# ChalmersPhotonicsLab/QAMpy

Hardware: AMD Instinct MI355X
Metric: equalised MSym/s (2-pol, 2 SPS) (higher is better)
Workload: dtype f32

## Files before the change

### qampy_amd/csrc/api.hip

```cpp
#include "common.h"
#include <stdlib.h>
#include <atomic>
#include <mutex>
#include <vector>
#include <unordered_map>
#include <string.h>

namespace qh {

thread_local hipStream_t g_stream = nullptr;
static thread_local hipStream_t g_streams[4] = {nullptr, nullptr, nullptr, nullptr};
int g_device = -1;
static thread_local std::string g_err;
static std::mutex g_mu;

void set_error(const std::string &s) { g_err = s; }

int hip_fail(hipError_t e, const char *what, const char *file, int line)
{
    g_err = std::string(hipGetErrorString(e)) + " in " + what + " (" + file + ":" + std::to_string(line) + ")";
    (void)hipGetLastError();
    return QH_ERR_HIP;
}

// ... 63 lines not shown
        QH_HIP(hipStreamCreateWithPriority(&g_streams[i], hipStreamNonBlocking, i == 2 ? prio_least : prio_greatest));
    }
    g_stream = g_streams[0];
    g_device = device;
    return QH_OK;
}

hipStream_t side_stream() { return g_stream == g_streams[0] ? g_streams[1] : g_streams[0]; }
hipStream_t helper_stream() { return g_streams[3]; }

int ensure_init()
{
    if (g_stream) return QH_OK;
    return init_device(g_device >= 0 ? g_device : 0);
}

thread_local void *g_scratch[SCRATCH_SLOTS] = {nullptr};
thread_local size_t g_scratch_n[SCRATCH_SLOTS] = {0};
thread_local unsigned g_scratch_epoch = 0;
static std::atomic<int> g_form[FORM_COUNT];
struct FormName { const char *key, *env; };
static const FormName FORM_NAMES[FORM_COUNT] = {
    {"trainer", "QAMPY_HIP_TRAINER"}, {"pit_form", "QAMPY_HIP_PIT_FORM"}, {"seg_lanes", "QAMPY_HIP_SEG_LANES"}, {"pit_probe", "QAMPY_HIP_PIT_PROBE"},
    {"bps", "QAMPY_HIP_BPS"}};
static int form_parse(int k, const char *v, int *out)
{
    if (!v || !v[0]) { *out = 0; return 0; }
    switch (k) {
    case FORM_TRAINER: *out = v[0] == 'd' ? 1 : (v[0] == 'l' ? 2 : (v[0] == 'i' ? 3 : (v[0] == 'a' || v[0] == '0' ? 0 : -1))); break;
    case FORM_PIT: *out = v[0] == 's' ? 1 : (v[0] == 'b' ? 2 : (v[0] == 'a' || v[0] == '0' ? 0 : -1)); break;
    case FORM_SEG_LANES: { const int n = atoi(v); *out = (n == 8 || n == 16 || n == 0) ? n : -1; break; }
    case FORM_BPS: *out = v[0] == 't' ? 1 : (v[0] == 'l' ? 2 : (v[0] == 'a' || v[0] == '0' ? 0 : -1)); break;
    default: *out = atoi(v) != 0 ? 1 : 0; break;
    }
    return *out < 0 ? -1 : 0;
}
static const int g_form_env_read = [] {
    for (int k = 0; k < FORM_COUNT; k++) {
        int v = 0;
        if (form_parse(k, getenv(FORM_NAMES[k].env), &v) == 0) g_form[k].store(v);
    }
    return 0;
}();
int form(FormKey k) { return g_form[k].load(std::memory_order_relaxed); }
const char *trainer_force()
{
    switch (form(FORM_TRAINER)) {
    case 1: return "direct";
    case 2: return "lookahead";
    case 3: return "iterative";
    default: return "";
    }
}
static constexpr int POOL_CLASSES = 48, POOL_KEEP = 8;
static constexpr size_t POOL_BYTES = (size_t)24 << 30;
// ... 370 lines not shown
```

### qampy_amd/csrc/common.h

```cpp
#pragma once
#include <hip/hip_runtime.h>
#include <stdint.h>
#include <string>
#include "../../include/qampy_hip.h"

namespace qh {

extern thread_local hipStream_t g_stream;
extern int g_device;
void set_error(const std::string &s);
int hip_fail(hipError_t e, const char *what, const char *file, int line);

#define QH_HIP(call)                                                        \
    do {                                                                    \
        hipError_t _e = (call);                                             \
        if (_e != hipSuccess) return qh::hip_fail(_e, #call, __FILE__, __LINE__); \
    } while (0)

#define QH_REQUIRE(cond, msg)                                   \
    do {                                                        \
        if (!(cond)) { qh::set_error(msg); return QH_ERR_ARG; } \
    } while (0)

#define QH_WAVE_FIRST() __builtin_amdgcn_s_setprio(3)

int ensure_init();
hipStream_t side_stream();
hipStream_t helper_stream();
enum FormKey { FORM_TRAINER = 0, FORM_PIT, FORM_SEG_LANES, FORM_PIT_PROBE, FORM_BPS, FORM_COUNT };
int form(FormKey k);
const char *trainer_force();
double gram_budget_gb();
int pit_timing_mode();
int default_tier();
double default_tier_tol();
constexpr int SCRATCH_SLOTS = 24;
constexpr int SCRATCH_TWOSTAGE = 16;
constexpr int SCRATCH_FOE = 17;
constexpr int SCRATCH_IMPAIR = 18;
constexpr int SCRATCH_PMD = 19;
constexpr int SCRATCH_TXRESP = 20;
constexpr int SCRATCH_SOS = 21;
constexpr int SCRATCH_CPR = 22;
constexpr int SCRATCH_FFT = 23;
int scratch(int slot, size_t bytes, void **p);
unsigned scratch_epoch();

int bps_twostage_recover_f32(const void *E, int nm, int64_t L, const void *angles, int A, int B, const void *symbols, int M, int N, int32_t *idx1,
                             int32_t *idx2, void *ph, void *Eout);
int bps_twostage_recover_f64(const void *E, int nm, int64_t L, const void *angles, int A, int B, const void *symbols, int M, int N, int32_t *idx1,
                             int32_t *idx2, void *ph, void *Eout);

// ... 114 lines not shown
```

### qampy_amd/csrc/train_pit.h

```cpp
#pragma once
#include <atomic>
#include <chrono>
#include <vector>
#include "train_impl.h"
#include "train_seg.h"

namespace qh {

typedef qh_pit_report PitCtrl;

constexpr double PIT_CONTRACT = 0.2;
constexpr int PIT_PROBE = 128;
constexpr int PIT_SEEDWIN = 512;
constexpr int PIT_MAXSEG = 65536;

__host__ __device__ inline int pit_symmetry(int method)
{
    switch (method) {
    case QH_M_CMA: case QH_M_SGNCMA: case QH_M_RDE: return 0;
    case QH_M_CMA2: return 2;
    default: return 4;
    }
}

// ... 832 lines not shown
                if (q < n) {
                    const float4 g = gch[rr * npair + lane];
                    const Zf up = row[p];
                    const Zf xqe = cmulf(Zf{g.z, -g.w}, row[q]);
                    row[p] = Zf{g.x * up.x - g.y * xqe.x, g.x * up.y - g.y * xqe.y};
                    row[q] = Zf{g.y * up.x + g.x * xqe.x, g.y * up.y + g.x * xqe.y};
                }
            }
            __builtin_amdgcn_fence(__ATOMIC_RELEASE, "wavefront");
        }
    }
    for (int k = lane; k < n; k += 64) { Vout[(size_t)i * n + k] = row[k]; Vout[(size_t)n * n + (size_t)k * n + i] = row[k]; }
}

constexpr int PIT_GT = 16, PIT_GC = PIT_GT / 8;
template <typename R> struct PitFuse {
    Cx<R> *X, *Y;
    const double *theta;
    const int64_t *modes_dev;
    int nmodes, nsel;
    float damp = 1.f;
    const Cx<R> *T2 = nullptr;
    float2 *Out2 = nullptr;
};
template <typename R, bool CONJT>
__global__ void __launch_bounds__(256) pit_cgemm_kernel(const Zf *A2, const Zf *B, Zf *C, int n, int ncol, const PitCtrl *c, PitFuse<R> fz)
{
    QH_WAVE_FIRST();
    if (c->done) return;
    extern __shared__ __attribute__((aligned(16))) char pit_smem[];
    Zf *As = reinterpret_cast<Zf *>(pit_smem);
    Zf *Bs = As + (size_t)PIT_EIGMAX * PIT_EIGMAX;
    const int tx = threadIdx.x & 7, ty = threadIdx.x >> 3;
    const int col0 = blockIdx.x * PIT_GT;
    const size_t wset = (size_t)fz.nmodes * n;
    for (int e = threadIdx.x; e < PIT_EIGMAX * n; e += 256) {
        const int k = e / PIT_EIGMAX, m = e - k * PIT_EIGMAX;
        Zf v{0.f, 0.f};
        if (m < n) { v = A2[(size_t)k * n + m]; if (CONJT) v.y = -v.y; }
        As[e] = v;
    }
    if (CONJT) {
        for (int e = threadIdx.x; e < n * PIT_GT; e += 256) {
            const int cc = e / n, k = e - cc * n, col = col0 + cc;
            Zf v{0.f, 0.f};
            if (col < ncol) {
// ... 233 lines not shown
            }
        } else if (threadIdx.x == 0) {
            float k11 = vals[0], k12 = vals[1], k22 = vals[2], zz = vals[3];
            const float cs = vals[4];
            const float n = cs > 0.f ? 1.f / cs : 0.f;
            k11 *= n; k12 *= n; k22 *= n; zz *= n;
            const float tr = 0.5f * (k11 + k22), df = 0.5f * (k11 - k22), rad = sqrtf(df * df + k12 * k12);
            float c = 1.f, sn = 0.f;
            if (rad > 1e-12f * (fabsf(tr) + 1e-30f)) { const float ang = 0.5f * atan2f(k12, df); c = cosf(ang); sn = sinf(ang); }
            PitModel m = a.model[j];
            m.k1 = tr + rad; m.k2 = tr - rad; m.q11 = c; m.q21 = sn; m.q12 = -sn; m.q22 = c; m.lam_u = zz;
            m.ok = (m.g > 0.f && m.g == m.g && m.k1 == m.k1 && m.k2 == m.k2) ? 1 : 0;
            a.model[j] = m;
        }
        __syncthreads();
    }
}

typedef float pit_f4 __attribute__((ext_vector_type(4)));
constexpr int PIT_MC = 16, PIT_MBP = PIT_MC + 1;
inline int pit_mfma_threads(int n) { return 64 * ((n + 15) / 16); }
inline size_t pit_mfma_lds(int n) { return ((size_t)(n + 4) * PIT_MBP + (size_t)PIT_MC * (PIT_EIGMAX + 1)) * sizeof(Zf); }
template <typename R, int MODE>
__global__ void __launch_bounds__(64 * (PIT_EIGMAX / 16)) pit_basis_mfma_kernel(const Zf *__restrict__ A2, const Cx<R> *__restrict__ T, const Zf *__restrict__ D, Zf *__restrict__ Out,
                                                                               int n, int ncol, const PitCtrl *c, PitFuse<R> fz)
{
    QH_WAVE_FIRST();
    if (c->done) return;
    extern __shared__ __attribute__((aligned(16))) char pit_smem[];
    const int np = (n + 3) & ~3;
    Zf *Bs = reinterpret_cast<Zf *>(pit_smem);
    Zf *Ct = Bs + (size_t)(n + 4) * PIT_MBP;
    const int tid = threadIdx.x, lane = tid & 63, wave = tid >> 6, nw = blockDim.x >> 6, nt = blockDim.x;
    const int nb1 = (ncol + PIT_MC - 1) / PIT_MC;
    const bool second = MODE == 0 && (int)blockIdx.x >= nb1;
    if (second) { T = fz.T2; Out = reinterpret_cast<Zf *>(fz.Out2); }
    const int col0 = ((int)blockIdx.x - (second ? nb1 : 0)) * PIT_MC;
    const size_t wset = (size_t)fz.nmodes * n;
    const int am = 16 * wave + (lane & 15), ak = lane >> 4;
    const Zf *ag = A2 + (size_t)ak * n + am;
    auto lda = [&](int k) -> Zf { return (am < n && k + ak < n) ? ag[(size_t)k * n] : Zf{0.f, 0.f}; };
    constexpr int PF = 8;
    Zf abuf[PF];
#pragma unroll
    for (int i = 0; i < PF; i++) abuf[i] = lda(4 * i);
    constexpr int NCW = 3;
    if (MODE == 0) {
        for (int cb = 0; cb < PIT_MC; cb += NCW * nw) {
            Zf tmp[NCW][2];
#pragma unroll
            for (int q = 0; q < NCW; q++) {
                const int cc = cb + wave + nw * q, col = col0 + cc;
                tmp[q][0] = Zf{0.f, 0.f}; tmp[q][1] = Zf{0.f, 0.f};
                if (cc < PIT_MC && col < ncol) {
                    const int s = col / fz.nsel, j = col - s * fz.nsel;
                    const Cx<R> *src = T + (size_t)s * wset + (size_t)fz.modes_dev[j] * n;
                    if (lane < n) { const Cx<R> t = src[lane]; tmp[q][0] = Zf{(float)t.re, (float)t.im}; }
                    if (lane + 64 < n) { const Cx<R> t = src[lane + 64]; tmp[q][1] = Zf{(float)t.re, (float)t.im}; }
                }
            }
// ... 70 lines not shown
    } else {
#pragma unroll
        for (int q = 0; q < 4; q++) {
            const int m = 16 * wave + 4 * (lane >> 4) + q;
            Ct[cl * (PIT_EIGMAX + 1) + m] = Zf{rr[q] - ii[q], im[q]};
        }
        __syncthreads();
        for (int cb = 0; cb < PIT_MC; cb += NCW * nw) {
#pragma unroll
            for (int q = 0; q < NCW; q++) {
                const int cc = cb + wave + nw * q, col = col0 + cc;
                if (cc < PIT_MC && col < ncol) {
                    const int s = col / fz.nsel, j = col - s * fz.nsel;
                    const size_t base = (size_t)s * wset + (size_t)fz.modes_dev[j] * n;
                    const double qr = pre ? th[q][0] : fz.theta[2 * (size_t)col], qi = pre ? th[q][1] : fz.theta[2 * (size_t)col + 1];
#pragma unroll
                    for (int h = 0; h < 2; h++) {
                        const int m = lane + 64 * h;
                        if (m < n) {
                            const Cx<R> x = pre ? xv[q][h] : fz.X[base + m];
                            const Zf d = Ct[cc * (PIT_EIGMAX + 1) + m];
                            const Cx<R> w{(R)(qr * x.re - qi * x.im + fz.damp * d.x), (R)(qr * x.im + qi * x.re + fz.damp * d.y)};
                            fz.X[base + m] = w;
                            fz.Y[base + m] = w;
                        }
                    }
                }
            }
        }
    }
}

static __global__ void __launch_bounds__(256) pit_bound_kernel(const Zf *Xe, const Zf *Ye, const Zf *Yprev, const double *lam, int n, int S, int nsel, int sym,
                                                              const PitCtrl *c, double *dfc, double *pw, double *gph, float4 *ualpha = nullptr)
{
    QH_WAVE_FIRST();
    if (c->done) return;
    const int lane = threadIdx.x & 63, bi = blockIdx.x * 4 + (threadIdx.x >> 6);
    const int nb = (S - 1) * nsel, ncol = S * nsel;
    if (bi >= nb + nsel) return;
    const bool result_probe = bi >= nb;
    const int j = result_probe ? bi - nb : bi % nsel;
    const int sb = result_probe ? S - 1 : bi / nsel;
    const Zf *pa = result_probe ? (c->passes == 0 ? Xe + (size_t)(S - 1) * nsel + j : Yprev + j) : Xe + (size_t)(sb + 1) * nsel + j;
    const size_t sa = (result_probe && c->passes != 0) ? (size_t)nsel : (size_t)ncol;
    const Zf *pb = Ye + (size_t)sb * nsel + j;
    Zf av[(PIT_EIGMAX + 63) / 64], bv[(PIT_EIGMAX + 63) / 64];
    float lv[(PIT_EIGMAX + 63) / 64];
    double A = 0, B = 0, Cr = 0, Ci = 0;
#pragma unroll
    for (int q = 0; q < (PIT_EIGMAX + 63) / 64; q++) {
        const int k = lane + 64 * q;
        av[q] = Zf{0.f, 0.f}; bv[q] = Zf{0.f, 0.f}; lv[q] = 0.f;
// ... 396 lines not shown
                const int s = s0 + q;
                run = cm(run, g[j][q]);
                if (s < s1) {
                    const double r = rsqrt(run.x * run.x + run.y * run.y);
                    th2[(size_t)s * nsel + j] = double2{run.x * r, run.y * r};
                }
            }
        }
        return;
    }
    for (int j = 0; j < nsel; j++) {
        double2 prod{1.0, 0.0};
        for (int s = s0; s < s1; s++)
            if (s > 0) prod = cm(prod, g2[(size_t)(s - 1) * nsel + j]);
        double2 run = block_scan_excl<double2, decltype(cm), NT>(prod, cm, double2{1.0, 0.0}, gbuf);
        for (int s = s0; s < s1; s++) {
            if (s > 0) run = cm(run, g2[(size_t)(s - 1) * nsel + j]);
            const double r = rsqrt(run.x * run.x + run.y * run.y);
            th2[(size_t)s * nsel + j] = double2{run.x * r, run.y * r};
        }
    }
}
template <typename R>
__global__ void __launch_bounds__(256) pit_devest_kernel(const Zf *D, const double *lam, int n, int ncol, const PitCtrl *c, float *devmax, unsigned *ticket, PitDecideArgs<R> da)
{
    QH_WAVE_FIRST();
    if (c->done) return;
    __shared__ float part[2][4][64], red[64], reds[64], redt[64], redm[64];
    const int cl = threadIdx.x & 63, kg = threadIdx.x >> 6;
    const int col = blockIdx.x * 64 + cl;
    float acc = 0.f, tap = 0.f;
    if (col < ncol) {
#pragma unroll 8
        for (int k = kg; k < n; k += 4) {
            const Zf v = D[(size_t)k * ncol + col];
            const float l = (float)lam[k], m2 = v.x * v.x + v.y * v.y;
            acc += (l > 0.f ? l : 0.f) * m2;
            tap += m2;
        }
    }
    part[0][kg][cl] = acc; part[1][kg][cl] = tap;
    __syncthreads();
    if (kg == 0) {
        acc = (part[0][0][cl] + part[0][1][cl]) + (part[0][2][cl] + part[0][3][cl]);
        tap = (part[1][0][cl] + part[1][1][cl]) + (part[1][2][cl] + part[1][3][cl]);
        red[cl] = (acc == acc) ? acc : 3.0e38f;
        reds[cl] = (acc == acc) ? acc : 3.0e38f;
        redt[cl] = (tap == tap) ? tap : 3.0e38f;
        redm[cl] = (tap == tap) ? tap : 3.0e38f;
    }
    __syncthreads();
    for (int s = 32; s > 0; s >>= 1) {
        if (threadIdx.x < s) {
            red[threadIdx.x] = red[threadIdx.x] > red[threadIdx.x + s] ? red[threadIdx.x] : red[threadIdx.x + s];
            reds[threadIdx.x] += reds[threadIdx.x + s];
            redt[threadIdx.x] += redt[threadIdx.x + s];
            redm[threadIdx.x] = redm[threadIdx.x] > redm[threadIdx.x + s] ? redm[threadIdx.x] : redm[threadIdx.x + s];
        }
        __syncthreads();
    }
    if (threadIdx.x == 0) {
        devmax[4 * blockIdx.x] = red[0]; devmax[4 * blockIdx.x + 1] = reds[0]; devmax[4 * blockIdx.x + 2] = redt[0]; devmax[4 * blockIdx.x + 3] = redm[0];
    }
    __shared__ int last;
    if (threadIdx.x == 0) {
        __threadfence();
        const unsigned t = atomicAdd(ticket, 1u);
        last = t == gridDim.x - 1;
        if (last) { *ticket = 0; __threadfence(); }
    }
    __syncthreads();
    if (!last) return;
    pit_decide_body<R>(da);
}
static __global__ void __launch_bounds__(256) pit_front_kernel(const Zf *D, const double *lam, int n, int ncol, double thr, int *front, int *bad)
{
    QH_WAVE_FIRST();
    const int col = blockIdx.x * 256 + threadIdx.x;
    if (col >= ncol) return;
    float acc = 0.f;
    for (int k = 0; k < n; k++) { const Zf v = D[(size_t)k * ncol + col]; const float l = (float)lam[k]; acc += (l > 0.f ? l : 0.f) * (v.x * v.x + v.y * v.y); }
    if (!(acc == acc) || acc > 1e30f) { atomicMax(bad, 1); return; }
    if ((double)acc > thr) atomicMax(front, col);
}
struct PitTiming { int npass; float pass_ms[QH_PIT_MAXPASS]; float acq_ms; };
inline PitTiming &pit_timing() { static thread_local PitTiming t; return t; }
constexpr int PIT_NEV = (QH_PIT_MAXPASS > QH_PIT_MAXCHUNK ? QH_PIT_MAXPASS : QH_PIT_MAXCHUNK) + 1;
struct PitEvents { hipEvent_t t0[PIT_NEV], t1[PIT_NEV], flag[PIT_NEV]; int32_t *hflag; float *hview; bool ok; };
inline PitEvents &pit_events()
{
    static thread_local PitEvents e = {{nullptr}, {nullptr}, {nullptr}, nullptr, nullptr, false};
    if (!e.ok) {
        for (int i = 0; i < PIT_NEV; i++) { (void)hipEventCreate(&e.t0[i]); (void)hipEventCreate(&e.t1[i]); (void)hipEventCreateWithFlags(&e.flag[i], hipEventDisableTiming); }
        (void)hipHostMalloc((void **)&e.hflag, PIT_NEV * sizeof(int32_t), hipHostMallocDefault);
        (void)hipHostMalloc((void **)&e.hview, 2 * PIT_NEV * sizeof(float), hipHostMallocCoherent);
        e.ok = e.hflag != nullptr && e.hview != nullptr;
// ... 395 lines not shown
    if (prepared) QH_REQUIRE(seg_form && o.acq_chunk > 0, "train_equaliser: a prepared acquisition belongs to throughput-form passes with acq_chunk given (qh_pit_prepare_*_dev said so)");
    if (block_form && !G && (!seg_form || amax > 0) && !prepared) {
        const int64_t n = seg_form ? pl.ngram : TrSyms;
        rc = pair_tab ? gram_build<R>(E, nmodes, L, os, ntaps, n, &G) : gram_cur_build<R>(E, nmodes, L, os, ntaps, n, &G);
        if (rc) return rc;
    }
    const int64_t g_per_step = pair_tab ? LA_B : GRAM_TRI / 2 / LA_B;

    const int ncol = sg.S * nsel;
    const double *lam = nullptr;
    const Zf *Vb = nullptr;
    Zf *Dz[2] = {nullptr, nullptr};
    Zf *Xe = nullptr, *Ye = nullptr, *Yprev = nullptr;
    if (want_corr) {
        void *cb = nullptr;
        if ((rc = scratch(10, pit_basis_bytes(ntot) + 4 * (size_t)ntot * ncol * sizeof(Zf) + (size_t)ntot * nsel * sizeof(Zf) + 256, &cb))) return rc;
        void *basis = o.basis ? o.basis : cb;
        if (!o.basis && (rc = pit_basis<R>(E, nmodes, L, os, ntaps, TrSyms, basis))) return rc;
        lam = (const double *)basis; Vb = (const Zf *)((const char *)basis + (size_t)ntot * sizeof(double));
        Dz[0] = (Zf *)((char *)cb + (pit_basis_bytes(ntot) + 63) / 64 * 64); Dz[1] = Dz[0] + (size_t)ntot * ncol;
        Xe = Dz[1] + (size_t)ntot * ncol; Ye = Xe + (size_t)ntot * ncol; Yprev = Ye + (size_t)ntot * ncol;
    }
    const bool eig = want_corr && sizeof(R) == 4 && form(FORM_PIT_PROBE) == 0;
    const bool tables_ok = method == QH_M_CMA || method == QH_M_SGNCMA || method == QH_M_MCMA || method == QH_M_RDE || method == QH_M_MRDE ||
                           (decision && (use_bi || seg_form));
    const bool ssb = eig && tables_ok && method != QH_M_CMA2;
    PitModel *model = nullptr;
    float4 *ualpha = nullptr;
    float2 *uqv = nullptr;
    PitModelArgs<R> ma;
    hipEvent_t model_event = nullptr;
    if (ssb) {
        void *mb = nullptr;
        const size_t pw_ = 2 * PIT_EIGMAX + 8;
        const size_t b_part = (size_t)PIT_MODB * 4 * nsel * pw_ * sizeof(float), b_u = ((size_t)nsel * ntot * sizeof(Cx<R>) + 63) / 64 * 64;
        const size_t b_ua = ((size_t)ncol * sizeof(float4) + 63) / 64 * 64, b_uq = ((size_t)ncol * sizeof(float2) + 63) / 64 * 64;
        if ((rc = scratch(14, b_part + b_u + b_ua + b_uq + 16 * sizeof(PitModel) + 128, &mb))) return rc;
        ma.part = (float *)mb; ma.u = (Cx<R> *)((char *)mb + b_part);
        ualpha = (float4 *)((char *)mb + b_part + b_u); uqv = (float2 *)((char *)ualpha + b_ua);
        model = (PitModel *)((char *)uqv + b_uq); ma.model = model; ma.ticket = (unsigned *)(model + 16);
        init.z[1] = ma.ticket; init.zn[1] = sizeof(unsigned);
        init.z[2] = ualpha; init.zn[2] = (unsigned)(b_ua + b_uq);
        ma.E = (const Cx<R> *)E; ma.wx = (const Cx<R> *)wx; ma.L = L; ma.TrSyms = TrSyms; ma.nmodes = nmodes; ma.ntaps = ntaps; ma.os = os; ma.nsel = nsel; ma.method = method;
        if (decision) { ma.symbols = (const Cx<R> *)f.dd_table; ma.nsy = 2 * f.dd_npart + 1; ma.sy_pitch = 2 * BI_DD_MAXLEV; ma.tables = 1; }
        else { ma.symbols = (const Cx<R> *)symbols; ma.nsy = nsy; ma.sy_pitch = nsy; ma.tables = (method == QH_M_RDE || method == QH_M_MRDE) ? 1 : 0; }
        for (int j = 0; j < 16; j++) ma.modes[j] = j < nsel ? modes[j] : 0;
        if (o.corr_beta < 0) beta = 0.0;
    }
    const size_t glds = ((size_t)PIT_EIGMAX * PIT_EIGMAX + (size_t)PIT_EIGMAX * PIT_GT) * sizeof(Zf);
    static std::atomic<bool> gemm_attr{false};
    if (want_corr && !gemm_attr.load(std::memory_order_acquire)) {
        QH_HIP(hipFuncSetAttribute((const void *)pit_cgemm_kernel<R, true>, hipFuncAttributeMaxDynamicSharedMemorySize, 160 * 1024 - 256));
        QH_HIP(hipFuncSetAttribute((const void *)pit_cgemm_kernel<R, false>, hipFuncAttributeMaxDynamicSharedMemorySize, 160 * 1024 - 256));
        QH_HIP(hipFuncSetAttribute((const void *)pit_basis_mfma_kernel<R, 0>, hipFuncAttributeMaxDynamicSharedMemorySize, 128 * 1024));
        QH_HIP(hipFuncSetAttribute((const void *)pit_basis_mfma_kernel<R, 1>, hipFuncAttributeMaxDynamicSharedMemorySize, 128 * 1024));
        gemm_attr.store(true, std::memory_order_release);
    }

    LaArgs<R> la = la_args<R>(E, L, nmodes, ntaps, os, modes, nsel, method, symbols, nsy, mu_dev, err, TrSyms * Niter);
    la.G = (const GramPair<R> *)G; la.gpair = pair_tab ? 1 : 0; la.wx_cs = (int64_t)wset;
    la.dd_general = f.dd_general;
    f.alphabet(la);
    const TrainArgs<R> ta = train_args<R>(E, L, nmodes, ntaps, os, TrSyms, Niter, modes, nsel, method, symbols, nsy, mu_dev, err);

    PitTiming &tm = pit_timing();
    tm.npass = 0; tm.acq_ms = 0;
    bool acq_timed = false;
    PitEvents &ev = pit_events();
    QH_REQUIRE(ev.ok, "train_equaliser: no pinned memory for the pass flags");
    const bool redo_ok = o.exact_redo_off == 0;
    bool fell_back = false;
    if (redo_ok && !adaptive) { init.cd[0] = w_call; init.cs[0] = wx; init.cn[0] = (unsigned)wbytes; }
    if (o.acquire && Niter > 0) { init.cd[1] = w_start; init.cs[1] = wx; init.cn[1] = (unsigned)wbytes; }
    hipLaunchKernelGGL(pit_init_kernel, dim3(32), dim3(256), 0, g_stream, init);
    QH_HIP(hipGetLastError());
    for (int it = 0; it < Niter; it++) {
        if (it == 0 && prepared) {
            const PitPrepLayout lay = pit_prep_layout<R>(nmodes, ntaps, amax);
// ... 42 lines not shown
            static thread_local hipEvent_t ev_seed = nullptr, ev_model = nullptr;
            if (!ev_seed) { QH_HIP(hipEventCreateWithFlags(&ev_seed, hipEventDisableTiming)); QH_HIP(hipEventCreateWithFlags(&ev_model, hipEventDisableTiming)); }
            hipStream_t ss = helper_stream();
            QH_HIP(hipEventRecord(ev_seed, g_stream));
            QH_HIP(hipStreamWaitEvent(ss, ev_seed, 0));
            hipLaunchKernelGGL((pit_model_kernel<R, 0>), dim3(PIT_MODB), dim3(256), 0, ss, ma);
            hipLaunchKernelGGL((pit_model_kernel<R, 1>), dim3(PIT_MODB), dim3(256), 0, ss, ma);
            QH_HIP(hipEventRecord(ev_model, ss));
            model_event = ev_model;
        }
        QH_HIP(hipGetLastError());
        const int timing_mode = pit_timing_mode();
        auto decide_args = [&](int p, const float *dm, const float2 *ye, float2 *yprev, int ne, int ncol_e, int corr_wanted) {
            PitDecideArgs<R> d;
            d.dfc = dfc; d.pw = pw; d.nb = (int)((sg.S - 1) * nsel); d.Ylast = (const Cx<R> *)(Y + (size_t)(sg.S - 1) * wset); d.n = (int)wset; d.wx = (Cx<R> *)wx; d.c = ctrl;
            d.host_view = &ev.hview[2 * p]; d.nrow = nsel; d.devmax = dm; d.ndev = ndev; d.safety = safety; d.Ye = ye; d.Yprev = yprev; d.ne = ne; d.ncol_e = ncol_e;
            d.theta = theta; d.modes_dev = (const int64_t *)modes_dev; d.ntot_w = ntot; d.S = (int)sg.S; d.sym = sym; d.corr_wanted = corr_wanted;
            d.extra = adaptive ? (const float *)ad_chg : nullptr;
            d.Dfin = (ye && !adaptive) ? (const float2 *)Dz[1] : nullptr; d.Vfin = (const float2 *)Vb; d.lam_fin = lam;
            d.stall_from = o.correction == 0 ? QH_PIT_MAXPASS : (adaptive ? 5 : 2);
            return d;
        };
        auto timed = [&](int p) { return timing_mode == 2 || (timing_mode == 1 && p == 1); };
        auto enqueue_pass = [&](int p) -> int {
            ((volatile float *)ev.hview)[2 * p] = -1.f;
            PitFuse<R> fz;
            fz.X = X; fz.Y = Y; fz.theta = theta; fz.modes_dev = (const int64_t *)modes_dev; fz.nmodes = nmodes; fz.nsel = nsel;
            fz.damp = (adaptive && p > 1) ? ad_damp : 1.f;
            if (p > 0 && want_corr) {
                if (eig)
                    hipLaunchKernelGGL((pit_basis_mfma_kernel<R, 1>), dim3((ncol + PIT_MC - 1) / PIT_MC), dim3(pit_mfma_threads(ntot)), pit_mfma_lds(ntot), g_stream, Vb + (size_t)ntot * ntot,
                                       (const Cx<R> *)nullptr, (const Zf *)Dz[1], (Zf *)nullptr, ntot, ncol, (const PitCtrl *)ctrl, fz);
                else
                    hipLaunchKernelGGL((pit_cgemm_kernel<R, false>), dim3((ncol + PIT_GT - 1) / PIT_GT), dim3(256), glds, g_stream, Vb + (size_t)ntot * ntot, (const Zf *)Dz[1], (Zf *)nullptr, ntot, ncol, (const PitCtrl *)ctrl, fz);
                QH_HIP(hipGetLastError());
            } else if (p > 0) {
                QH_HIP(hipMemcpyAsync(X + wset, Y, (size_t)(sg.S - 1) * wbytes, hipMemcpyDeviceToDevice, g_stream));
                QH_HIP(hipMemcpyAsync(Y, X, (size_t)sg.S * wbytes, hipMemcpyDeviceToDevice, g_stream));
            }
            if (o.on_pass) {
                hipStream_t keep = g_stream;
                o.on_pass(o.on_pass_user, it, p);
                g_stream = keep;
            }
            if (timed(p)) QH_HIP(hipEventRecord(ev.t0[p], g_stream));
            if (seg_form) {
                SegArgs<R> sa{};
                sa.E = (const Cx<R> *)E; sa.wx = Y; sa.symbols = la.symbols; sa.err = (Cx<R> *)err; sa.mu = mu_dev;
                sa.L = L; sa.TrSyms = TrSyms; sa.nsy = la.nsy; sa.sy_pitch = la.sy_pitch; sa.err_pitch = TrSyms * Niter; sa.err_off = (int64_t)it * TrSyms;
                sa.nmodes = nmodes; sa.ntaps = ntaps; sa.os = os; sa.nsel = nsel; sa.S = sg.S;
                sa.seg_len = sg.len; sa.seg_extra = sg.extra; sa.seg_tail = sg.tail; sa.seg_begin = sg.begin;
                sa.r_in = ad_rS; sa.r_out = ad_rE; sa.e_in = ad_eS; sa.e_out = ad_eE; sa.mu_sum = (R *)ad_M; sa.adapt_first = sg.begin > 0 ? 1 : 0;
                for (int j = 0; j < 16; j++) sa.modes[j] = j < nsel ? modes[j] : 0;
                sa.skip = &ctrl->done;
                sa.q_first = own_first * nsel; sa.q_count = split ? own_count * nsel : 0;
                pit_last_launch().form = 1;
                if (!split || own_count > 0) { int r = launch_seg<R>(sa, method, adaptive); if (r) return r; }
                if (adaptive) hipLaunchKernelGGL((pit_adapt_scan_kernel<R>), dim3(1), dim3(1024), 0, g_stream, ad_rS, (const R *)ad_rE, ad_eS, (const Cx<R> *)ad_eE, sg.S, ad_chg, (const PitCtrl *)ctrl, ad_relax, ad_rP, ad_dP, ad_newton);
            } else if (block_form) {
                LaArgs<R> ls = la;
                ls.TrSyms = sg.len; ls.nch = sg.S; ls.wx = Y; ls.err_off = (int64_t)it * TrSyms; ls.seg = 1; ls.seg_extra = sg.extra; ls.seg_tail = sg.tail;
                ls.skip = &ctrl->done;
                pit_last_launch() = PitLaunch{use_bi ? 2 : 3, 0, 0, 0, 0, 0};
                if (sg.begin > 0) {
                    ls.E = (const Cx<R> *)E + sg.begin * os; ls.L = L - sg.begin * os; ls.err_off += sg.begin;
                    ls.G = (const GramPair<R> *)G + sg.begin * g_per_step;
                }
                { int r = use_bi ? launch_bi<R>(ls) : launch_la<R>(ls); if (r) return r; }
            } else {
                TrainArgs<R> ts = ta;
                ts.wx = Y; ts.nseg = sg.S; ts.seg_begin = sg.begin; ts.seg_len = sg.len; ts.seg_extra = sg.extra; ts.seg_tail = sg.tail; ts.seg_iter = it; ts.skip = &ctrl->done;
// ... 9 lines not shown
                if (o.exchange(o.exchange_user, Y, (size_t)sg.S * wbytes) != 0) { set_error("train_equaliser: the exchange callback failed"); return QH_ERR_ARG; }
            }
            const int nbnd = (int)((sg.S - 1) * nsel);
            if (eig) {
                if (o.basis && pit_basis_sync().pending) {
                    QH_HIP(hipStreamWaitEvent(g_stream, pit_basis_sync().out, 0));
                    pit_basis_sync().pending = false;
                }
                auto forward2 = [&](const Cx<R> *src, Zf *dst, const Cx<R> *src2, Zf *dst2) {
                    PitFuse<R> f2 = fz;
                    f2.T2 = src2; f2.Out2 = reinterpret_cast<float2 *>(dst2);
                    hipLaunchKernelGGL((pit_basis_mfma_kernel<R, 0>), dim3(2 * ((ncol + PIT_MC - 1) / PIT_MC)), dim3(pit_mfma_threads(ntot)), pit_mfma_lds(ntot), g_stream, Vb, src, (const Zf *)nullptr, dst, ntot, ncol, (const PitCtrl *)ctrl, f2);
                };
                if (p == 0 && model_event) QH_HIP(hipStreamWaitEvent(g_stream, model_event, 0));
                forward2((const Cx<R> *)X, Xe, (const Cx<R> *)Y, Ye);
                hipLaunchKernelGGL(pit_bound_kernel, dim3((nbnd + nsel + 3) / 4), dim3(256), 0, g_stream, (const Zf *)Xe, (const Zf *)Ye, (const Zf *)Yprev, lam, ntot, sg.S, nsel, sym,
                                   (const PitCtrl *)ctrl, dfc, pw, gph, ualpha);
                hipLaunchKernelGGL((pit_gauge_kernel<R>), dim3(ssb ? 2 : 1), dim3(PIT_GT_THREADS), 0, g_stream, (const double *)gph, sg.S, nsel, ctrl, theta, (const double *)pw,
                                   nbnd, method, (const Cx<R> *)symbols + (size_t)modes[0] * nsy, 1, (const PitModel *)model, (const float4 *)ualpha, uqv,
                                   (const R *)mu_dev, sg.len, (const float *)ad_M);
                hipLaunchKernelGGL((pit_recur_eig_kernel<R>), dim3(ntot, nsel), dim3(PIT_RT), 0, g_stream, Xe, (const Zf *)Ye, Dz[1], (const double *)theta, lam, nsel, sg.S, sg.len,
                                   (const R *)mu_dev, beta, (const PitCtrl *)ctrl, (const float *)ad_M, (adaptive && p >= 1) ? ad_damp : 1.f,
                                   (const float4 *)ualpha, (const float2 *)uqv);
                hipLaunchKernelGGL((pit_devest_kernel<R>), dim3(ndev), dim3(256), 0, g_stream, (const Zf *)Dz[1], lam, ntot, ncol, (const PitCtrl *)ctrl, devmax, ticket,
                                   decide_args(p, (const float *)devmax, (const float2 *)Ye, (float2 *)Yprev, ntot, ncol, 1));
            } else {
            const size_t dlds = (2 * (size_t)ntot + (size_t)nmodes * os * pit_phase_pitch(ntaps, os, PIT_PROBE)) * sizeof(Cx<R>);
            QH_REQUIRE(dlds <= 60 * 1024, "train_equaliser: boundary probe does not fit the LDS for this filter shape");
            hipLaunchKernelGGL((pit_defect_kernel<R>), dim3(sg.S, nsel), dim3(PIT_PROBE), dlds, g_stream, (const Cx<R> *)E, nmodes, L, os,
                               ntaps, sg, TrSyms, (const int64_t *)modes_dev, (const Cx<R> *)X, (const Cx<R> *)Y, sym, (const PitCtrl *)ctrl, dfc, pw, gph, (const Cx<R> *)wx);
            hipLaunchKernelGGL((pit_gauge_kernel<R>), dim3(1), dim3(PIT_GT_THREADS), 0, g_stream, (const double *)gph, sg.S, nsel, ctrl, theta, (const double *)pw,
                               nbnd, method, (const Cx<R> *)symbols + (size_t)modes[0] * nsy, want_corr ? 1 : 0);
            if (want_corr) {
                if (o.basis && pit_basis_sync().pending) {
                    QH_HIP(hipStreamWaitEvent(g_stream, pit_basis_sync().out, 0));
                    pit_basis_sync().pending = false;
                }
                hipLaunchKernelGGL((pit_cgemm_kernel<R, true>), dim3((ncol + PIT_GT - 1) / PIT_GT), dim3(256), glds, g_stream, Vb, (const Zf *)nullptr, Dz[1], ntot, ncol, (const PitCtrl *)ctrl, fz);
                hipLaunchKernelGGL((pit_recur_kernel<R>), dim3(ntot, nsel), dim3(256), 0, g_stream, Dz[1], lam, nsel, sg.S, sg.len, (const R *)mu_dev, beta, (const PitCtrl *)ctrl);
                hipLaunchKernelGGL((pit_devest_kernel<R>), dim3(ndev), dim3(256), 0, g_stream, (const Zf *)Dz[1], lam, ntot, ncol, (const PitCtrl *)ctrl, devmax, ticket,
                                   decide_args(p, (const float *)devmax, (const float2 *)nullptr, (float2 *)nullptr, 0, 0, 1));
            } else
                hipLaunchKernelGGL((pit_decide_kernel<R>), dim3(1), dim3(256), 0, g_stream, decide_args(p, (const float *)nullptr, (const float2 *)nullptr, (float2 *)nullptr, 0, 0, 0));
            }
            QH_HIP(hipGetLastError());
            return QH_OK;
// ... 157 lines not shown
```

### qampy_amd/csrc/train_seg.h

```cpp
#pragma once
#include "train_bi.h"

namespace qh {

constexpr int SG_CH = 64;

template <typename R> struct SegArgs {
    const Cx<R> *E;
    Cx<R> *wx;
    const Cx<R> *symbols;
    Cx<R> *err;
    const R *mu;
    int64_t L, TrSyms, nsy, sy_pitch, err_pitch, err_off;
    int nmodes, ntaps, os, nsel, S;
    int64_t seg_len, seg_extra, seg_tail, seg_begin;
    int64_t modes[16];
    const int *skip;
    int q_first, q_count;
    int lpm, pitch, rag, nslots;
    int ch;
    const R *r_in; R *r_out; const Cx<R> *e_in; Cx<R> *e_out; R *mu_sum; int adapt_first;
};

__device__ __forceinline__ void row16_csum(float &re, float &im)
{
    asm volatile(
        "s_nop 1\n\t"
        "v_add_f32_dpp %0, %0, %0 quad_perm:[1,0,3,2] row_mask:0xf bank_mask:0xf\n\t"
        "v_add_f32_dpp %1, %1, %1 quad_perm:[1,0,3,2] row_mask:0xf bank_mask:0xf\n\t"
        "s_nop 0\n\t"
        "v_add_f32_dpp %0, %0, %0 quad_perm:[2,3,0,1] row_mask:0xf bank_mask:0xf\n\t"
        "v_add_f32_dpp %1, %1, %1 quad_perm:[2,3,0,1] row_mask:0xf bank_mask:0xf\n\t"
// ... 253 lines not shown
    const int nq = a.q_count > 0 ? a.q_first + a.q_count : a.S * a.nsel;
    const int q0 = a.q_first + blockIdx.x * CPW;
    const int q = q0 + lane / LPC;
    const bool alive = q < nq;
    const int qc = alive ? q : nq - 1;
    const int seg = qc / a.nsel, jsel = qc - seg * a.nsel;
    const int seg0 = q0 / a.nsel;
    const int segl = ((q0 + CPW - 1 < nq ? q0 + CPW - 1 : nq - 1)) / a.nsel;
    const int nslot = segl - seg0 + 1;
    const int slot = seg - seg0;
    const int mode = (int)a.modes[jsel];
    const int ntot = a.nmodes * a.ntaps;
    const int os_ = a.os;
    auto seg_start = [&](int64_t s) { return a.seg_begin + s * a.seg_len + (s < a.seg_extra ? s : a.seg_extra) * LA_B; };
    auto seg_steps = [&](int64_t s) { return (int)(a.seg_len + (s < a.seg_extra ? LA_B : 0) + (s == a.S - 1 ? a.seg_tail : 0)); };
    const int64_t my_start = seg_start(seg);
    const int my_steps = alive ? seg_steps(seg) : 0;
    int max_steps = 0, min_steps = 0x7fffffff;
    for (int s = seg0; s <= segl; s++) { const int n = seg_steps(s); max_steps = n > max_steps ? n : max_steps; min_steps = n < min_steps ? n : min_steps; }
    if (q0 + CPW - 1 >= nq) min_steps = 0;

    const int kin = l16 / a.lpm, t0 = (l16 - kin * a.lpm) * TPL;
    const bool has = kin < a.nmodes;
    Cx<R> *wrow = a.wx + ((size_t)seg * a.nmodes + mode) * ntot;
    v2 w[TPL];
#pragma unroll
    for (int j = 0; j < TPL; j++) {
        const bool ok = has && t0 + j < a.ntaps;
        const Cx<R> v = ok ? wrow[kin * a.ntaps + t0 + j] : Cx<R>{0, 0};
        w[j] = v2{v.re, v.im};
    }
    const Cx<R> *sy = a.symbols + (size_t)mode * a.sy_pitch;
    LaConst<R, NPART> K;
    K.mu = *a.mu;
    { const Cx<R> c0 = sy[0]; K.R_re = c0.re; K.R_im = c0.im; }
    K.code0_re = K.R_re; K.code0_im = K.R_im;
    tab_fill<R, NPART>(K.tab, sy, 0, NPART + 1);
    LaConst<R, NPART> Ks = K;
    Ks.code0_re *= K.mu; Ks.code0_im *= K.mu;
    tab_scale_codes<R, NPART>(Ks.tab, K.mu);
    R ad_r = 1, ad_sum = 0;
    Cx<R> ad_ep{0, 0};
    bool ad_skip0 = false;
    if constexpr (ADAPT) { ad_r = a.r_in[qc]; ad_ep = a.e_in[qc]; ad_skip0 = a.adapt_first == 0 && my_start == 0; }

    constexpr int rowsz = PITCH;
    constexpr int bufsz = SG_ROWS * PITCH;
// ... 225 lines not shown
        if (c + 1 < nchunk) stage_load(c + 1);
        const Cx<R> *xs = has ? lds + (slot * a.nmodes + kin) * rowsz + t0 : zero_row;
        const int xstep = has ? os_ : 0;
        const int ibase = c * CH;
        const int nst = (max_steps - ibase) < CH ? (max_steps - ibase) : CH;
        auto run2 = [&](auto RG, auto OS2) __attribute__((always_inline)) {
            if (ibase + nst <= min_steps) run_chunk(xs, xstep, ibase, nst, SgInt<0>{}, RG, OS2);
            else run_chunk(xs, xstep, ibase, nst, SgInt<1>{}, RG, OS2);
        };
        auto run = [&](auto RG) __attribute__((always_inline)) {
            if (os_ == 2) run2(RG, SgInt<1>{}); else run2(RG, SgInt<0>{});
        };
        switch (rag) {
        case 0: run(SgInt<0>{}); break;
        case 1: run(SgInt<1>{}); break;
        case 2: run(SgInt<(TPL > 2 ? 2 : 0)>{}); break;
        default: run(SgInt<(TPL > 3 ? 3 : 0)>{}); break;
        }
        __syncthreads();
        if (c + 1 < nchunk) stage_store(c + 1);
        __syncthreads();
    }
    if (alive) {
#pragma unroll
        for (int j = 0; j < TPL; j++)
            if (has && t0 + j < a.ntaps) stg(wrow + kin * a.ntaps + t0 + j, Cx<R>{w[j].x, w[j].y});
        if constexpr (ADAPT) if (l16 == 0) { a.r_out[q] = ad_r; a.e_out[q] = ad_ep; a.mu_sum[q] = ad_sum; }
    }
}

#endif

inline int seg_tpl(int nmodes, int ntaps, int lpc = 16)
{
    for (int tpl : {2, 4, 6, 8, 11}) {
        if (lpc == 16 ? tpl == 11 : (tpl != 6 && tpl != 11)) continue;
        const int lpm = (ntaps + tpl - 1) / tpl;
        if (nmodes * lpm <= lpc && lpm * tpl - ntaps <= SG_MAXRAG && lpm * tpl - ntaps < tpl) return tpl;
    }
    return 0;
}
inline int seg_slots(int nsel, int cpw = 4)
{
    int n = 1;
    for (int q0 = 0; q0 <= cpw * nsel; q0 += cpw) { const int m = (q0 + cpw - 1) / nsel - q0 / nsel + 1; n = m > n ? m : n; }
    return n;
}
inline bool seg_supported(int method, int nmodes, int ntaps, int os, int64_t nsy, size_t elem, int nsel = 1, int rows = 4)
{
// ... 163 lines not shown
```

Before: 1202.

## Fuse PIT deviation-estimate and next-pass basis product into one tail kernel

Adds a pit_tail_kernel that runs the devest reduction/decide blocks and the next pass's MFMA basis-product blocks in a single launch. When this path is active, the next pass skips its separate basis launch. The basis product writes only X, and the segment kernel reads weights from X and writes its results to Y, which removes a duplicate Y store. This saves one launch and one serialization point per pass. The trade-off is that the basis product is now computed speculatively before the decide step, and the launch uses a larger block size with big LDS for all blocks, which may lower occupancy for the devest blocks.

New measurement: 1240, median of 6. 3.2% higher.

```diff
diff --git a/qampy_amd/csrc/api.hip b/qampy_amd/csrc/api.hip
--- a/qampy_amd/csrc/api.hip
+++ b/qampy_amd/csrc/api.hip
@@ -109,7 +109,7 @@
 struct FormName { const char *key, *env; };
 static const FormName FORM_NAMES[FORM_COUNT] = {
     {"trainer", "QAMPY_HIP_TRAINER"}, {"pit_form", "QAMPY_HIP_PIT_FORM"}, {"seg_lanes", "QAMPY_HIP_SEG_LANES"}, {"pit_probe", "QAMPY_HIP_PIT_PROBE"},
-    {"bps", "QAMPY_HIP_BPS"}};
+    {"bps", "QAMPY_HIP_BPS"}, {"pit_tail", "QAMPY_HIP_PIT_TAIL"}};
 static int form_parse(int k, const char *v, int *out)
 {
     if (!v || !v[0]) { *out = 0; return 0; }
@@ -118,6 +118,7 @@
     case FORM_PIT: *out = v[0] == 's' ? 1 : (v[0] == 'b' ? 2 : (v[0] == 'a' || v[0] == '0' ? 0 : -1)); break;
     case FORM_SEG_LANES: { const int n = atoi(v); *out = (n == 8 || n == 16 || n == 0) ? n : -1; break; }
     case FORM_BPS: *out = v[0] == 't' ? 1 : (v[0] == 'l' ? 2 : (v[0] == 'a' || v[0] == '0' ? 0 : -1)); break;
+    case FORM_PIT_TAIL: *out = v[0] == 's' ? 1 : (v[0] == 'a' || v[0] == '0' ? 0 : -1); break;
     default: *out = atoi(v) != 0 ? 1 : 0; break;
     }
     return *out < 0 ? -1 : 0;
diff --git a/qampy_amd/csrc/common.h b/qampy_amd/csrc/common.h
--- a/qampy_amd/csrc/common.h
+++ b/qampy_amd/csrc/common.h
@@ -27,7 +27,7 @@
 int ensure_init();
 hipStream_t side_stream();
 hipStream_t helper_stream();
-enum FormKey { FORM_TRAINER = 0, FORM_PIT, FORM_SEG_LANES, FORM_PIT_PROBE, FORM_BPS, FORM_COUNT };
+enum FormKey { FORM_TRAINER = 0, FORM_PIT, FORM_SEG_LANES, FORM_PIT_PROBE, FORM_BPS, FORM_PIT_TAIL, FORM_COUNT };
 int form(FormKey k);
 const char *trainer_force();
 double gram_budget_gb();
diff --git a/qampy_amd/csrc/train_pit.h b/qampy_amd/csrc/train_pit.h
--- a/qampy_amd/csrc/train_pit.h
+++ b/qampy_amd/csrc/train_pit.h
@@ -878,6 +878,7 @@
     float damp = 1.f;
     const Cx<R> *T2 = nullptr;
     float2 *Out2 = nullptr;
+    int x_only = 0;
 };
 template <typename R, bool CONJT>
 __global__ void __launch_bounds__(256) pit_cgemm_kernel(const Zf *A2, const Zf *B, Zf *C, int n, int ncol, const PitCtrl *c, PitFuse<R> fz)
@@ -1157,20 +1158,18 @@
 inline int pit_mfma_threads(int n) { return 64 * ((n + 15) / 16); }
 inline size_t pit_mfma_lds(int n) { return ((size_t)(n + 4) * PIT_MBP + (size_t)PIT_MC * (PIT_EIGMAX + 1)) * sizeof(Zf); }
 template <typename R, int MODE>
-__global__ void __launch_bounds__(64 * (PIT_EIGMAX / 16)) pit_basis_mfma_kernel(const Zf *__restrict__ A2, const Cx<R> *__restrict__ T, const Zf *__restrict__ D, Zf *__restrict__ Out,
-                                                                               int n, int ncol, const PitCtrl *c, PitFuse<R> fz)
-{
-    QH_WAVE_FIRST();
-    if (c->done) return;
+__device__ __forceinline__ void pit_basis_mfma_body(const Zf *__restrict__ A2, const Cx<R> *__restrict__ T, const Zf *__restrict__ D, Zf *__restrict__ Out,
+                                                    int n, int ncol, const PitFuse<R> &fz, const int bid, const int nt)
+{
     extern __shared__ __attribute__((aligned(16))) char pit_smem[];
     const int np = (n + 3) & ~3;
     Zf *Bs = reinterpret_cast<Zf *>(pit_smem);
     Zf *Ct = Bs + (size_t)(n + 4) * PIT_MBP;
-    const int tid = threadIdx.x, lane = tid & 63, wave = tid >> 6, nw = blockDim.x >> 6, nt = blockDim.x;
+    const int tid = threadIdx.x, lane = tid & 63, wave = tid >> 6, nw = nt >> 6;
     const int nb1 = (ncol + PIT_MC - 1) / PIT_MC;
-    const bool second = MODE == 0 && (int)blockIdx.x >= nb1;
+    const bool second = MODE == 0 && bid >= nb1;
     if (second) { T = fz.T2; Out = reinterpret_cast<Zf *>(fz.Out2); }
-    const int col0 = ((int)blockIdx.x - (second ? nb1 : 0)) * PIT_MC;
+    const int col0 = (bid - (second ? nb1 : 0)) * PIT_MC;
     const size_t wset = (size_t)fz.nmodes * n;
     const int am = 16 * wave + (lane & 15), ak = lane >> 4;
     const Zf *ag = A2 + (size_t)ak * n + am;
@@ -1287,13 +1286,21 @@
                             const Zf d = Ct[cc * (PIT_EIGMAX + 1) + m];
                             const Cx<R> w{(R)(qr * x.re - qi * x.im + fz.damp * d.x), (R)(qr * x.im + qi * x.re + fz.damp * d.y)};
                             fz.X[base + m] = w;
-                            fz.Y[base + m] = w;
+                            if (!fz.x_only) fz.Y[base + m] = w;
                         }
                     }
                 }
             }
         }
     }
+}
+template <typename R, int MODE>
+__global__ void __launch_bounds__(64 * (PIT_EIGMAX / 16)) pit_basis_mfma_kernel(const Zf *__restrict__ A2, const Cx<R> *__restrict__ T, const Zf *__restrict__ D, Zf *__restrict__ Out,
+                                                                               int n, int ncol, const PitCtrl *c, PitFuse<R> fz)
+{
+    QH_WAVE_FIRST();
+    if (c->done) return;
+    pit_basis_mfma_body<R, MODE>(A2, T, D, Out, n, ncol, fz, (int)blockIdx.x, (int)blockDim.x);
 }
 
 static __global__ void __launch_bounds__(256) pit_bound_kernel(const Zf *Xe, const Zf *Ye, const Zf *Yprev, const double *lam, int n, int S, int nsel, int sym,
@@ -1736,13 +1743,12 @@
     }
 }
 template <typename R>
-__global__ void __launch_bounds__(256) pit_devest_kernel(const Zf *D, const double *lam, int n, int ncol, const PitCtrl *c, float *devmax, unsigned *ticket, PitDecideArgs<R> da)
-{
-    QH_WAVE_FIRST();
-    if (c->done) return;
+__device__ __forceinline__ void pit_devest_body(const Zf *D, const double *lam, int n, int ncol, float *devmax, unsigned *ticket, const PitDecideArgs<R> &da,
+                                                const int bid, const int nblk)
+{
     __shared__ float part[2][4][64], red[64], reds[64], redt[64], redm[64];
     const int cl = threadIdx.x & 63, kg = threadIdx.x >> 6;
-    const int col = blockIdx.x * 64 + cl;
+    const int col = bid * 64 + cl;
     float acc = 0.f, tap = 0.f;
     if (col < ncol) {
 #pragma unroll 8
@@ -1774,18 +1780,39 @@
         __syncthreads();
     }
     if (threadIdx.x == 0) {
-        devmax[4 * blockIdx.x] = red[0]; devmax[4 * blockIdx.x + 1] = reds[0]; devmax[4 * blockIdx.x + 2] = redt[0]; devmax[4 * blockIdx.x + 3] = redm[0];
+        devmax[4 * bid] = red[0]; devmax[4 * bid + 1] = reds[0]; devmax[4 * bid + 2] = redt[0]; devmax[4 * bid + 3] = redm[0];
     }
     __shared__ int last;
     if (threadIdx.x == 0) {
         __threadfence();
         const unsigned t = atomicAdd(ticket, 1u);
-        last = t == gridDim.x - 1;
+        last = t == (unsigned)nblk - 1;
         if (last) { *ticket = 0; __threadfence(); }
     }
     __syncthreads();
     if (!last) return;
     pit_decide_body<R>(da);
+}
+template <typename R>
+__global__ void __launch_bounds__(256) pit_devest_kernel(const Zf *D, const double *lam, int n, int ncol, const PitCtrl *c, float *devmax, unsigned *ticket, PitDecideArgs<R> da)
+{
+    QH_WAVE_FIRST();
+    if (c->done) return;
+    pit_devest_body<R>(D, lam, n, ncol, devmax, ticket, da, (int)blockIdx.x, (int)gridDim.x);
+}
+template <typename R>
+__global__ void __launch_bounds__(64 * (PIT_EIGMAX / 16)) pit_tail_kernel(const Zf *__restrict__ D, const double *lam, int n, int ncol, const PitCtrl *c, float *devmax, unsigned *ticket,
+                                                                         int ndev, PitDecideArgs<R> da, const Zf *__restrict__ VT, PitFuse<R> fz, int nt_prod)
+{
+    QH_WAVE_FIRST();
+    if (c->done) return;
+    if ((int)blockIdx.x < ndev) {
+        if (threadIdx.x >= 256) return;
+        pit_devest_body<R>(D, lam, n, ncol, devmax, ticket, da, (int)blockIdx.x, ndev);
+    } else {
+        if ((int)threadIdx.x >= nt_prod) return;
+        pit_basis_mfma_body<R, 1>(VT, (const Cx<R> *)nullptr, D, (Zf *)nullptr, n, ncol, fz, (int)blockIdx.x - ndev, nt_prod);
+    }
 }
 static __global__ void __launch_bounds__(256) pit_front_kernel(const Zf *D, const double *lam, int n, int ncol, double thr, int *front, int *bad)
 {
@@ -2227,6 +2254,7 @@
         Xe = Dz[1] + (size_t)ntot * ncol; Ye = Xe + (size_t)ntot * ncol; Yprev = Ye + (size_t)ntot * ncol;
     }
     const bool eig = want_corr && sizeof(R) == 4 && form(FORM_PIT_PROBE) == 0;
+    const bool tail_fused = eig && seg_form && !adaptive && !split && form(FORM_PIT_TAIL) == 0;
     const bool tables_ok = method == QH_M_CMA || method == QH_M_SGNCMA || method == QH_M_MCMA || method == QH_M_RDE || method == QH_M_MRDE ||
                            (decision && (use_bi || seg_form));
     const bool ssb = eig && tables_ok && method != QH_M_CMA2;
@@ -2259,6 +2287,7 @@
         QH_HIP(hipFuncSetAttribute((const void *)pit_cgemm_kernel<R, false>, hipFuncAttributeMaxDynamicSharedMemorySize, 160 * 1024 - 256));
         QH_HIP(hipFuncSetAttribute((const void *)pit_basis_mfma_kernel<R, 0>, hipFuncAttributeMaxDynamicSharedMemorySize, 128 * 1024));
         QH_HIP(hipFuncSetAttribute((const void *)pit_basis_mfma_kernel<R, 1>, hipFuncAttributeMaxDynamicSharedMemorySize, 128 * 1024));
+        QH_HIP(hipFuncSetAttribute((const void *)pit_tail_kernel<R>, hipFuncAttributeMaxDynamicSharedMemorySize, 128 * 1024));
         gemm_attr.store(true, std::memory_order_release);
     }
 
@@ -2347,12 +2376,15 @@
             return d;
         };
         auto timed = [&](int p) { return timing_mode == 2 || (timing_mode == 1 && p == 1); };
+        int back_done_for = 0;
         auto enqueue_pass = [&](int p) -> int {
             ((volatile float *)ev.hview)[2 * p] = -1.f;
             PitFuse<R> fz;
             fz.X = X; fz.Y = Y; fz.theta = theta; fz.modes_dev = (const int64_t *)modes_dev; fz.nmodes = nmodes; fz.nsel = nsel;
             fz.damp = (adaptive && p > 1) ? ad_damp : 1.f;
-            if (p > 0 && want_corr) {
+            fz.x_only = tail_fused ? 1 : 0;
+            if (p > 0 && tail_fused && back_done_for == p) {
+            } else if (p > 0 && want_corr) {
                 if (eig)
                     hipLaunchKernelGGL((pit_basis_mfma_kernel<R, 1>), dim3((ncol + PIT_MC - 1) / PIT_MC), dim3(pit_mfma_threads(ntot)), pit_mfma_lds(ntot), g_stream, Vb + (size_t)ntot * ntot,
                                        (const Cx<R> *)nullptr, (const Zf *)Dz[1], (Zf *)nullptr, ntot, ncol, (const PitCtrl *)ctrl, fz);
@@ -2371,7 +2403,7 @@
             if (timed(p)) QH_HIP(hipEventRecord(ev.t0[p], g_stream));
             if (seg_form) {
                 SegArgs<R> sa{};
-                sa.E = (const Cx<R> *)E; sa.wx = Y; sa.symbols = la.symbols; sa.err = (Cx<R> *)err; sa.mu = mu_dev;
+                sa.E = (const Cx<R> *)E; sa.wx = tail_fused ? X : Y; sa.wx_out = tail_fused ? Y : nullptr; sa.symbols = la.symbols; sa.err = (Cx<R> *)err; sa.mu = mu_dev;
                 sa.L = L; sa.TrSyms = TrSyms; sa.nsy = la.nsy; sa.sy_pitch = la.sy_pitch; sa.err_pitch = TrSyms * Niter; sa.err_off = (int64_t)it * TrSyms;
                 sa.nmodes = nmodes; sa.ntaps = ntaps; sa.os = os; sa.nsel = nsel; sa.S = sg.S;
                 sa.seg_len = sg.len; sa.seg_extra = sg.extra; sa.seg_tail = sg.tail; sa.seg_begin = sg.begin;
@@ -2427,6 +2459,15 @@
                 hipLaunchKernelGGL((pit_recur_eig_kernel<R>), dim3(ntot, nsel), dim3(PIT_RT), 0, g_stream, Xe, (const Zf *)Ye, Dz[1], (const double *)theta, lam, nsel, sg.S, sg.len,
                                    (const R *)mu_dev, beta, (const PitCtrl *)ctrl, (const float *)ad_M, (adaptive && p >= 1) ? ad_damp : 1.f,
                                    (const float4 *)ualpha, (const float2 *)uqv);
+                if (tail_fused) {
+                    const int nt_prod = pit_mfma_threads(ntot);
+                    PitFuse<R> fn = fz;
+                    fn.damp = 1.f;
+                    hipLaunchKernelGGL((pit_tail_kernel<R>), dim3(ndev + (ncol + PIT_MC - 1) / PIT_MC), dim3(nt_prod > 256 ? nt_prod : 256), pit_mfma_lds(ntot), g_stream,
+                                       (const Zf *)Dz[1], lam, ntot, ncol, (const PitCtrl *)ctrl, devmax, ticket, ndev,
+                                       decide_args(p, (const float *)devmax, (const float2 *)Ye, (float2 *)Yprev, ntot, ncol, 1), Vb + (size_t)ntot * ntot, fn, nt_prod);
+                    back_done_for = p + 1;
+                } else
                 hipLaunchKernelGGL((pit_devest_kernel<R>), dim3(ndev), dim3(256), 0, g_stream, (const Zf *)Dz[1], lam, ntot, ncol, (const PitCtrl *)ctrl, devmax, ticket,
                                    decide_args(p, (const float *)devmax, (const float2 *)Ye, (float2 *)Yprev, ntot, ncol, 1));
             } else {
diff --git a/qampy_amd/csrc/train_seg.h b/qampy_amd/csrc/train_seg.h
--- a/qampy_amd/csrc/train_seg.h
+++ b/qampy_amd/csrc/train_seg.h
@@ -8,6 +8,7 @@
 template <typename R> struct SegArgs {
     const Cx<R> *E;
     Cx<R> *wx;
+    Cx<R> *wx_out;
     const Cx<R> *symbols;
     Cx<R> *err;
     const R *mu;
@@ -307,7 +308,8 @@
 
     const int kin = l16 / a.lpm, t0 = (l16 - kin * a.lpm) * TPL;
     const bool has = kin < a.nmodes;
-    Cx<R> *wrow = a.wx + ((size_t)seg * a.nmodes + mode) * ntot;
+    const size_t woff = ((size_t)seg * a.nmodes + mode) * ntot;
+    const Cx<R> *wrow = a.wx + woff;
     v2 w[TPL];
 #pragma unroll
     for (int j = 0; j < TPL; j++) {
@@ -579,9 +581,10 @@
         __syncthreads();
     }
     if (alive) {
+        Cx<R> *wend = (a.wx_out ? a.wx_out : a.wx) + woff;
 #pragma unroll
         for (int j = 0; j < TPL; j++)
-            if (has && t0 + j < a.ntaps) stg(wrow + kin * a.ntaps + t0 + j, Cx<R>{w[j].x, w[j].y});
+            if (has && t0 + j < a.ntaps) stg(wend + kin * a.ntaps + t0 + j, Cx<R>{w[j].x, w[j].y});
         if constexpr (ADAPT) if (l16 == 0) { a.r_out[q] = ad_r; a.e_out[q] = ad_ep; a.mu_sum[q] = ad_sum; }
     }
 }
```
